# jiahuei/COMIC-Compact-Image-Captioning-with-Attention

Hardware: AMD Instinct MI355X
Metric: images/sec (decoder-mode XE training, COMIC-256, InceptionV3 frozen) (higher is better)
Workload: dtype bf16

## Files before the change

### comic-compact-image-captioning-with-attention_amd/_lib.py

```python
import ctypes as C
import os

_HERE = os.path.dirname(os.path.abspath(__file__))
LIB_PATH = os.environ.get('COMIC_HIP_LIB') or os.path.join(_HERE, 'lib', 'libcomic_hip.so')

c_void_p, c_int, c_int32, c_int64, c_float, c_double, c_char_p, c_uint64 = (
    C.c_void_p, C.c_int, C.c_int32, C.c_int64, C.c_float, C.c_double, C.c_char_p, C.c_uint64)


class CnnOp(C.Structure):
    _fields_ = [(n, c_int32) for n in (
        'kind', 'src', 'dst', 'src_coff', 'dst_coff', 'H', 'W', 'Cin', 'Cout', 'KH', 'KW', 'SH', 'SW',
        'PT', 'PL', 'Ho', 'Wo', 'weight', 'relu', 'out_f32', 'src_f32', 'lane', 'tile', 'group', 'flags', 'min_lds')]


class ImageDesc(C.Structure):
    _fields_ = [('offset', C.c_int64), ('in_h', c_int32), ('in_w', c_int32), ('flip', c_int32), ('oy', c_int32),
                ('ox', c_int32), ('sy', C.c_float), ('sx', C.c_float)]


class ConvWeight(C.Structure):
    _fields_ = [('w', c_void_p), ('scale', c_void_p), ('shift', c_void_p), ('w_frag', c_void_p)]


# ... 7 lines not shown
        'init_method', 'start_id', 'end_id')] + [(n, c_float) for n in (
            'keep_in', 'keep_out', 'keep_alpha', 'map_loss_scale')] + [('flags', C.c_uint32),
                                                                       ('length_penalty_weight', c_float),
                                                                       ('cell', c_int32)]


CELLS = {'LSTM': 0, 'LN_LSTM': 1, 'GRU': 2}


(DEC_NO_PERSIST, DEC_NO_PERSIST_BWD, DEC_NO_FUSED_STEP, DEC_NO_SPLIT_ATTN_BWD, DEC_ONE_LANE, DEC_EXACT_GEMM, DEC_STAMPS,
 DEC_NO_BEAM_LOGITS, DEC_NO_LSTM_STREAM) = (1, 2, 4, 8, 16, 32, 64, 128, 256)
DEC_PHASE_FWD, DEC_PHASE_BWD = 512, 1024
DEC_NO_GROUP_GEMM = 2048
DEC_BWD_OWN_ROWS = 4096
DEC_INJECT_TIMEOUT = 8192
CNN_BWD_NO_ACT_FUSION = 2
_DEC_ENV = (('COMIC_PERSIST', '0', DEC_NO_PERSIST), ('COMIC_PERSIST_BWD', '0', DEC_NO_PERSIST_BWD),
            ('COMIC_FUSED_STEP', '0', DEC_NO_FUSED_STEP), ('COMIC_SPLIT_ATTN_BWD', '0', DEC_NO_SPLIT_ATTN_BWD),
            ('COMIC_GRAD_LANES', '0', DEC_ONE_LANE), ('COMIC_SPLIT3', '0', DEC_EXACT_GEMM),
            ('COMIC_PERSIST_STAMPS', '1', DEC_STAMPS), ('COMIC_BEAM_LOGITS', '0', DEC_NO_BEAM_LOGITS),
            ('COMIC_LSTM_STREAM', '0', DEC_NO_LSTM_STREAM), ('COMIC_GROUP_GEMM', '0', DEC_NO_GROUP_GEMM),
            ('COMIC_BWD_OWN_ROWS', '1', DEC_BWD_OWN_ROWS))


def decoder_flags_from_env():
    f = 0
    for name, val, bit in _DEC_ENV:
        if os.environ.get(name, '')[:1] == val:
            f |= bit
    return f
# ... 77 lines not shown
    'comic_xent_fwd_bwd': (c_int, [P, P, P, P, P, P, P, P, c_int, c_int, c_int, P]),
    'comic_argmax_rows': (c_int, [P, P, c_int, c_int, P]),
    'comic_beam_step': (c_int, [P, P, P, P, P, P, P, c_int, c_int, c_int, c_int, P]),
    'comic_gather_rows': (c_int, [P, P, P, c_int, c_int, c_int, P]),
    'comic_gather_tree': (c_int, [P, P, P, P, c_int, c_int, c_int, c_int, P]),
    'comic_adam_tf': (c_int, [P, P, P, P, c_int64, c_float, c_float, c_float, c_float, c_float, c_float, P]),
    'comic_adam_tf_gated': (c_int, [P, P, P, P, c_int64, c_float, c_float, c_float, c_float, c_float, c_float, P, P]),
    'comic_momentum_tf_gated': (c_int, [P, P, P, c_int64, c_float, c_float, c_float, c_float, P, P]),
    'comic_debug_occupy_cus': (c_int, [c_int, c_int, P]),
    'comic_colsum': (c_int, [P, P, c_int, c_int, c_float, P]),
    'comic_ln_tanh_fwd': (c_int, [P, P, P, P, P, c_int, c_int, c_float, P]),
    'comic_ln_tanh_bwd_rows': (c_int, [P, P, P, P, P, c_int, c_int, P]),
    'comic_momentum_tf': (c_int, [P, P, P, c_int64, c_float, c_float, c_float, c_float, P]),
    'comic_axpy': (c_int, [P, P, c_float, c_int64, P]),
    'comic_decoder_train_workspace': (c_int64, [P, c_int, c_int]),
    'comic_decoder_train_path': (c_int, []),
    'comic_decoder_greedy_path': (c_int, []),
    'comic_decoder_beam_path': (c_int, []),
    'comic_beam_step_dense_workspace': (c_int64, [c_int, c_int, c_int, c_int]),
    'comic_beam_step_dense': (c_int, [c_void_p] * 9 + [c_int] * 5 + [c_void_p, c_int64, c_void_p]),
    'comic_gemm_f32_stream_workspace': (c_int64, [c_int, c_int, c_int]),
    'comic_gemm_f32_stream': (c_int, [c_void_p, c_void_p, c_void_p, c_void_p, c_int, c_int, c_int, c_void_p, c_int64, c_void_p]),
    'comic_decoder_infer_workspace': (c_int64, [P, c_int, c_int]),
    'comic_decoder_train_step': (c_int, [P, P, P, P, P, P, P, P, P, P, c_int, c_int, c_int, P, P, P, P, P, P, P,
                                         P, P, P, P, P, c_int64, P]),
    'comic_decoder_greedy': (c_int, [P, P, P, P, c_int, c_int, P, P, P, P, P, c_int64, P]),
    'comic_decoder_sample': (c_int, [P, P, P, P, c_int, c_int, P, P, P, P, P, P, c_int64, P]),
    'comic_decoder_beam': (c_int, [P, P, P, P, c_int, c_int, c_int, P, P, P, P, P, P, P, P, c_int64, P]),
    'comic_scorer_create': (c_void_p, [c_char_p, P, c_int64, c_double]),
    'comic_scorer_destroy': (None, [c_void_p]),
# ... 106 lines not shown
```

### comic-compact-image-captioning-with-attention_amd/csrc/decoder_exec.hip

```cpp
#include <atomic>
#include <stdlib.h>

#include <algorithm>
#include <string.h>

#include "common.h"
#include "decoder_math.h"
#include "decoder_persist.h"
#include "gemm_group.h"
#include "lstm_prep.h"
#include "lstm_stream_dev.h"

int comic_gemm_f32_ws(const float* A, const float* B, float* C, const float* bias, int M, int N, int K, int lda,
                      int ldb, int ldc, int trans_a, int trans_b, float alpha, float beta, void* ws, int64_t ws_bytes,
                      hipStream_t st);
int comic_xent_ex(float* logits, const int32_t* targets_bt, const float* coef_bt, const float* wmask_bt,
                  const int32_t* lens, float* loss_rows, float* dlogits, int32_t* ids_tb, int t_rows, int t_stride,
                  int B, int V, hipStream_t st);

int comic_attn_fwd_ex(const comic_attn_desc* d, const float* keys, const float* values, const float* q,
                      const float* ln_g, const float* ln_b, const float* v, const float* tau, const float* mask_alpha,
                      float keep_alpha, float* alpha, float* alpha_d, float* ctx, const int32_t* lens, int t,
                      const float* att_prev, float* att_next, float* xh_next, int xh_ld, const float* mask_next,
                      int mask_ld, float keep_in, int q_parts, float* q_out, float* scores_ws, hipStream_t st,
// ... 770 lines not shown
  w.take<unsigned>(kPersistSyncWords + kGroupTickets);
  w.take<float>(TB * 4 * D); w.take<float>((long)T * ((B + 15) / 16) * 16 * 4 * D);
  w.take<float>((long)T * ((B + 15) / 16) * 16 * D);
  w.take<float>(TB * 2 * D);
  w.take<float>(4 * B * (3 * D + 1));
  w.take<float>(TB * 64);
  if (comic_persist_fwd_bigm((int)M, d->fm_projection == 2)) w.take<float>(TB * 8 * M);
  if (d->cell == COMIC_CELL_LN_LSTM) {
    w.take<float>((TB + B) * 5 * D); w.take<float>((TB + B) * 8); w.take<float>((TB + B) * 10 * D); w.take<float>(10 * D);
  } else if (d->cell == COMIC_CELL_GRU) {
    w.take<float>(TB * Wd); w.take<float>(2 * B * Wd); w.take<float>(4 * D);
  }
  return (int64_t)w.off;
}

extern "C" int comic_decoder_train_step(const comic_decoder_desc* d, const comic_decoder_params* p,
                                        const comic_decoder_params* gr, const float* fm, const float* im_embed,
                                        const int32_t* inputs_bt, const int32_t* targets_bt, const float* wmask_bt,
                                        const float* coef_bt, const int32_t* lens, int B, int T, int Tp,
                                        const float* mask_init_in, const float* mask_in, const float* mask_out,
                                        const float* mask_alpha, float* logits_tb, int32_t* ids_tb, float* attn_hist,
                                        float* loss_rows, float* map_loss, float* dfm, float* dim_embed,
                                        void* workspace, int64_t workspace_bytes, void* stream) {
  RC(check_desc(d));
  FlagScope flag_scope__(d);
  COMIC_REQUIRE(p && gr && fm && im_embed && inputs_bt && targets_bt && wmask_bt && coef_bt && lens,
                "train_step: null input");
  COMIC_REQUIRE(logits_tb && ids_tb && attn_hist && loss_rows && map_loss && workspace, "train_step: null output");
  COMIC_REQUIRE(B > 0 && T > 0 && Tp > 0 && Tp <= T, "train_step: bad B/T/Tp (%d %d %d)", B, T, Tp);
  COMIC_REQUIRE(workspace_bytes >= comic_decoder_train_workspace(d, B, T), "train_step: workspace too small");
  COMIC_REQUIRE(d->keep_in >= 1.f || (mask_in && (d->init_method == 1 || mask_init_in)),
                "train_step: input dropout enabled but no mask given");
  COMIC_REQUIRE(d->keep_out >= 1.f || mask_out, "train_step: output dropout enabled but no mask given");
  COMIC_REQUIRE(d->keep_alpha >= 1.f || mask_alpha, "train_step: attention dropout enabled but no mask given");
  hipStream_t st = (hipStream_t)stream;
  const int D = d->D, E = d->E, A = d->A, V = d->V, M = d->M, H = d->H, Cv = d->Cv, EA = E + A, Wd = E + A + D;
  const long TB = (long)T * B;
  const bool drop_in = d->keep_in < 1.f, drop_out = d->keep_out < 1.f, drop_al = d->keep_alpha < 1.f;
  Bump w(workspace, (size_t)workspace_bytes);
  float* keys = w.take<float>((long)B * M * D);
  float* values_buf = w.take<float>((long)B * M * D);
  InitBufs ib;
  ib.x = w.take<float>((long)B * EA); ib.xh = w.take<float>((long)B * EA);
  ib.g = w.take<float>((long)B * 4 * D); ib.gates = w.take<float>((long)B * 4 * D); ib.c_new = w.take<float>((long)B * D);
  float* emb_all = w.take<float>(TB * E);
// ... 82 lines not shown
    if (persist_b) {
      pr.p[3] = dq_part; pr.n[3] = (long)Tp * B * 4 * D;
      pr.p[4] = dg_blk; pr.n[4] = 4 * n16;
      pr.p[5] = dstate; pr.n[5] = (long)Tp * B * 2 * D;
      pr.p[6] = dq_sum; pr.n[6] = n16;
      pr.p[7] = dotp; pr.n[7] = (long)Tp * B * 64;
    }
    ComicPrologueExtra px{};
    prologue_rides = group_gemm_enabled() && cell == COMIC_CELL_LSTM && fused;
    if (prologue_rides) {
      px.K = p->K; px.panel = kpanel_f; px.D = D; px.Wd = Wd; px.n_pack = comic_lstm_panel_floats(D, Wd, 0);
      if (Vp != V) { px.W_o = p->W_o; px.wo_pad = wo_pad; px.V = V; px.Vp = Vp; px.n_pad = (long)D * Vp; }
    }
    RC(comic_persist_prepare(pr, persist_sync, kPersistSyncWords + kGroupTickets, st, prologue_rides ? &px : nullptr));
  }
  const bool grp = group_gemm_enabled() && cell == COMIC_CELL_LSTM && (long)Tp * B >= 64 && (long)B * M >= 64 && B >= 16;
  const int ldl = grp ? Vp : V;
  const float* wo_g = (grp && Vp != V) ? wo_pad : p->W_o;
  float* xh_init = xh_all + (size_t)Tp * B * Wd;
  float* dg_init = dg_all + (size_t)Tp * B * 4 * D;
  void* const gg_slab = g_splitk_ws;
  const int64_t gg_slab_cap = 2 * kSplitKBytes;
  SideLane* L = grp ? nullptr : side_lane();
  if (do_fwd) {
  if (grp) {
    if (!persist) COMIC_REQUIRE(hipMemsetAsync(gg_tickets, 0, sizeof(unsigned) * kGroupTickets, st) == hipSuccess, "train_step: memset");
    if (fused && !(prologue_rides && persist_b)) RC(comic_pack_lstm_panels(p->K, prologue_rides ? nullptr : kpanel_f, persist_b ? nullptr : kpanel_b, D, Wd, st));
    if (fused_q && !persist_b) RC(comic_pack_wq_panel(p->W_q, wq_panel, D, st));
    if (Vp != V && !prologue_rides) {
      const long n = (long)D * Vp;
      hipLaunchKernelGGL(pad_rows_kernel, dim3((unsigned)cdiv64(n, 256)), dim3(256), 0, st, p->W_o, wo_pad, V, Vp, n);
      COMIC_LAUNCH_CHECK("pad W_o");
    }
    GemmGroupRun g1;
    g1.add(COMIC_GG_NN, fm, p->W_m, keys, B * M, D, d->C, d->C, D, D);
    if (d->fm_projection == 1) g1.add(COMIC_GG_NN, fm, p->W_v, values_buf, B * M, D, d->C, d->C, D, D);
    if (d->init_method == 1) {
      g1.add(COMIC_GG_NN, im_embed, p->W_init, hs, B, D, d->Cg, d->Cg, D, D);
    } else {
      ComicGemmProb* q = g1.add(COMIC_GG_NN, im_embed, p->W_init, xh_init, B, EA, d->Cg, d->Cg, EA, Wd);
      if (drop_in) { q->mask = mask_init_in; q->ld_mask = EA; q->keep = d->keep_in; }
    }
    RC(g1.run(gg_slab, gg_slab_cap, gg_tickets, st));
    if (d->init_method == 1) {
      RC(fill(cs, 0.f, (long)B * D, st));
    } else {
      GemmGroupRun g2;
      g2.add(COMIC_GG_NN, xh_init, p->K, ib.g, B, 4 * D, EA, Wd, 4 * D, 4 * D)->bias = p->b;
      RC(g2.run(gg_slab, gg_slab_cap, gg_tickets, st));
    }
  } else {
    LaneScope lane(L, st, splitk_ws_b);
    RC(lane.rc);
    hipStream_t sl = lane.lane();
    if (fused) RC(comic_pack_lstm_panels(p->K, kpanel_f, persist_b ? nullptr : kpanel_b, D, Wd, sl));
// ... 239 lines not shown
      hipLaunchKernelGGL(input_bwd_kernel, dim3(cdiv(B * Wd, 256)), dim3(256), 0, st, part,
                         drop_in ? mask_in + (size_t)t * B * EA : nullptr, d->keep_in, demb + (size_t)t * B * E,
                         datt, dh, lens, t, carry, B, E, A, D, S4);
      COMIC_LAUNCH_CHECK("input_bwd");
    }
  }
  float* dx_im = nullptr;
  int n_init = 0;
  if (grp) {
    const bool init_step = d->init_method != 1;
    const int rows_k = (Tp + (init_step ? 1 : 0)) * B;
    if (init_step)
      RC(comic_lstm_gates_bwd(ib.gates, nullptr, ib.c_new, nullptr, nullptr, 1.f, nullptr, 0, dc, dh, dg_init, B, D, (void*)st));
    GemmGroupRun g1, g2;
    g1.add(COMIC_GG_TN, xh_all, dg_all, gr->K, Wd, 4 * D, rows_k, Wd, 4 * D, 4 * D);
    g1.add(COMIC_GG_TN, fm, dkeys, gr->W_m, d->C, D, B * M, d->C, D, D);
    if (d->fm_projection == 1) g1.add(COMIC_GG_TN, fm, dvalues_buf, gr->W_v, d->C, D, B * M, d->C, D, D);
    if (persist_b) {
      ComicGemmProb* q = g1.add(COMIC_GG_NT, dg_all, p->K, demb, Tp * B, E, 4 * D, 4 * D, 4 * D, E);
      if (drop_in) { q->mask = mask_in; q->ld_mask = EA; q->keep = d->keep_in; }
    }
    g1.add(COMIC_GG_TN, y_all, dq_all, gr->W_q, D, D, Tp * B, D, D, D);
    g1.add(COMIC_GG_TN, y_all, dlogits, gr->W_o, D, V, Tp * B, D, ldl, V);
    if (dfm) g1.add(COMIC_GG_NT, dkeys, p->W_m, dfm, B * M, d->C, D, D, D, d->C);
    g1.add_colsum(dg_all, gr->b, 4 * D, rows_k, 4 * D);
    g1.add_colsum(dlogits, gr->b_o, V, Tp * B, ldl);
    if (d->method == 0) {
      const float* pg = persist_b ? pgrad4 : pgrad;
      const int pr = persist_b ? 4 * B : Tp * B, ldp = 3 * D + 1;
      g1.add_colsum(pg, gr->v, D, pr, ldp);
      g1.add_colsum(pg + D, gr->ln_g, D, pr, ldp);
      g1.add_colsum(pg + 2 * D, gr->ln_b, D, pr, ldp);
      g1.add_colsum(pg + 3 * D, gr->tau, 1, pr, ldp);
    }
    if (init_step) {
      ComicGemmProb* q = g1.add(COMIC_GG_NT, dg_init, p->K, dx_init, B, EA, 4 * D, 4 * D, 4 * D, EA);
      if (drop_in) { q->mask = mask_init_in; q->ld_mask = EA; q->keep = d->keep_in; }
      dx_im = dx_init;
      n_init = EA;
      g2.add(COMIC_GG_TN, im_embed, dx_im, gr->W_init, d->Cg, n_init, B, d->Cg, n_init, n_init);
      if (dim_embed) g2.add(COMIC_GG_NT, dx_im, p->W_init, dim_embed, B, d->Cg, n_init, n_init, n_init, d->Cg);
    } else {
      dx_im = dh;
      n_init = D;
      g1.add(COMIC_GG_TN, im_embed, dx_im, gr->W_init, d->Cg, n_init, B, d->Cg, n_init, n_init);
      if (dim_embed) g1.add(COMIC_GG_NT, dx_im, p->W_init, dim_embed, B, d->Cg, n_init, n_init, n_init, d->Cg);
    }
    if (d->fm_projection == 1 && dfm) {
      ComicGemmProb* q = g2.add(COMIC_GG_NT, dvalues_buf, p->W_v, dfm, B * M, d->C, D, D, D, d->C);
      q->beta = 1.f;
    }
    RC(g1.run(gg_slab, gg_slab_cap, gg_tickets, st));
    RC(comic_embed_bwd_set(in_tb, demb, gr->emb, Tp * B, E, V, st));
    RC(g2.run(gg_slab, gg_slab_cap, gg_tickets, st));
    if (d->fm_projection == 0 && dfm) RC(comic_axpy(dfm, dvalues_buf, 1.f, (int64_t)B * M * Cv, (void*)st));
  } else {
  LaneScope glane(L, st, splitk_ws_b);
  RC(glane.rc);
  hipStream_t sb = glane.lane();
  RC(gemm_big(y_all, dlogits, gr->W_o, nullptr, D, V, Tp * B, D, V, V, 1, 0, 0.f, sb));
// ... 531 lines not shown
```

### comic-compact-image-captioning-with-attention_amd/csrc/gemm_group.h

```cpp
#pragma once
#include "common.h"

constexpr int kGemmGroupMax = 20;
enum { COMIC_GG_TN = 0, COMIC_GG_NN = 1, COMIC_GG_NT = 2 };

struct ComicGemmProb {
  const float* A;
  const float* B;
  float* C;
  const float* bias;
  const float* mask;
  int M, N, K, lda, ldb, ldc, ld_mask;
  float alpha, beta;
  float keep;
  int type;
  int ones_a;
  int tiles_m, tiles_n, S, k_per_slice, wg_begin;
  int slab_tile0;
  int ticket0;
};

struct ComicGemmGroup {
  ComicGemmProb p[kGemmGroupMax];
  int n;
  float* slab;
  unsigned* tickets;
  int xcd_chunk;
};

int comic_gemm_group_plan(ComicGemmGroup& g, int target_items, int64_t* slab_bytes, int* n_tickets);
constexpr int kGemmGroupTargetItems = 640;
// ... 2 lines not shown
```

### comic-compact-image-captioning-with-attention_amd/csrc/gemm_group.hip

```cpp
#include <algorithm>

#include "gemm_group.h"
#include "gemm_x3_dev.h"

namespace {

constexpr int GB = 128;
constexpr int kGemmGroupSlots = 512;
constexpr int kItemOverhead = 6;
constexpr int kSc1 = 16;
typedef __attribute__((ext_vector_type(4))) unsigned gg_u32x4_t;

__device__ __forceinline__ __amdgpu_buffer_rsrc_t gg_rsrc(const void* p, long bytes) {
  return __builtin_amdgcn_make_buffer_rsrc((void*)p, 0, (int)bytes, 0x00020000);
}
__device__ __forceinline__ float4 gg_load16_sc1(__amdgpu_buffer_rsrc_t r, unsigned off) {
  const gg_u32x4_t v = __builtin_amdgcn_raw_buffer_load_b128(r, (int)off, 0, kSc1);
  return make_float4(__uint_as_float(v.x), __uint_as_float(v.y), __uint_as_float(v.z), __uint_as_float(v.w));
}
__device__ __forceinline__ void gg_store16_sc1(__amdgpu_buffer_rsrc_t r, unsigned off, float4 v) {
  const gg_u32x4_t u = {__float_as_uint(v.x), __float_as_uint(v.y), __float_as_uint(v.z), __float_as_uint(v.w)};
  __builtin_amdgcn_raw_buffer_store_b128(u, r, (int)off, 0, kSc1);
}

// ... 67 lines not shown
    red[kg * 32 + cg] = sm;
    __syncthreads();
    if (tid < 32) {
      float4 tot = red[cg];
#pragma unroll
      for (int k = 1; k < KG; ++k) {
        const float4 v = red[k * 32 + cg];
        tot.x += v.x; tot.y += v.y; tot.z += v.z; tot.w += v.w;
      }
      if (S == 1) gg_emit(p, 0, n, tot);
      else gg_store16_sc1(sr, sbase + (unsigned)cg * 16u, tot);
    }
    if (S == 1) return;
  } else {
    f32x4_t acc[4][4];
    if constexpr (PC) {
      if (p.type == COMIC_GG_TN) x3_mainloop_pc<false, false>(p.A, p.B, p.M, p.N, p.lda, p.ldb, m0, n0, kbeg, kend, smem, acc);
      else if (p.type == COMIC_GG_NN) x3_mainloop_pc<true, false>(p.A, p.B, p.M, p.N, p.lda, p.ldb, m0, n0, kbeg, kend, smem, acc);
      else x3_mainloop_pc<true, true>(p.A, p.B, p.M, p.N, p.lda, p.ldb, m0, n0, kbeg, kend, smem, acc);
    } else {
      if (p.type == COMIC_GG_TN)
        x3_mainloop<GB, false, false, GB>(p.A, p.B, p.M, p.N, p.lda, p.ldb, m0, n0, kbeg, kend, smem, acc);
      else if (p.type == COMIC_GG_NN)
        x3_mainloop<GB, true, false, GB>(p.A, p.B, p.M, p.N, p.lda, p.ldb, m0, n0, kbeg, kend, smem, acc);
      else
        x3_mainloop<GB, true, true, GB>(p.A, p.B, p.M, p.N, p.lda, p.ldb, m0, n0, kbeg, kend, smem, acc);
    }
    const bool owner = wave < 4;
    if (S == 1) {
      if (owner)
#pragma unroll
      for (int i = 0; i < 4; ++i)
#pragma unroll
        for (int j = 0; j < 4; ++j)
          gg_emit(p, m0 + wm * 64 + j * 16 + (lane & 15), n0 + wn * 64 + i * 16 + (lane >> 4) * 4,
                  make_float4(acc[i][j][0], acc[i][j][1], acc[i][j][2], acc[i][j][3]));
      return;
    }
    if (owner)
#pragma unroll
    for (int i = 0; i < 4; ++i)
// ... 35 lines not shown
    }
  }
}


}

int comic_gemm_group_plan(ComicGemmGroup& g, int target_items, int64_t* slab_bytes, int* n_tickets) {
  COMIC_REQUIRE(g.n > 0 && g.n <= kGemmGroupMax, "gemm_group: %d problems", g.n);
  long cost = 0;
  for (int i = 0; i < g.n; ++i) {
    ComicGemmProb& p = g.p[i];
    COMIC_REQUIRE(p.M > 0 && p.N > 0 && p.K > 0 && p.B && p.C && (p.A || p.ones_a), "gemm_group: bad problem %d", i);
    COMIC_REQUIRE(p.type >= COMIC_GG_TN && p.type <= COMIC_GG_NT, "gemm_group: bad type of problem %d", i);
    COMIC_REQUIRE(!p.ones_a || (p.type == COMIC_GG_TN && p.M == 1), "gemm_group: ones_a needs type TN and M = 1 (problem %d)", i);
    COMIC_REQUIRE(p.ldc >= p.N && (!p.mask || p.ld_mask >= p.N), "gemm_group: leading dimension of problem %d", i);
    if (!p.ones_a) COMIC_REQUIRE(p.lda >= (p.type == COMIC_GG_TN ? p.M : p.K), "gemm_group: lda of problem %d", i);
    COMIC_REQUIRE(p.ldb >= (p.type == COMIC_GG_NT ? p.K : p.N), "gemm_group: ldb of problem %d", i);
    p.tiles_m = cdiv(p.M, GB);
    p.tiles_n = cdiv(p.N, GB);
    cost += (long)cdiv(p.M, GB) * p.tiles_n * cdiv(p.K, 32);
  }
  auto split_of = [](int kt, long klen) { return (int)std::min<long>(16, std::max<long>(1, (kt + klen / 2) / klen)); };
  long klen = std::max<long>(8, cost / std::max(1, target_items));
  {
    long best = -1, best_klen = klen, kt_max = 8;
    for (int i = 0; i < g.n; ++i) kt_max = std::max<long>(kt_max, cdiv(g.p[i].K, 32));
    for (long kl = klen; kl <= kt_max; ++kl) {
      long items = 0, longest = 0;
      for (int i = 0; i < g.n; ++i) {
// ... 29 lines not shown
  }
  if (slab_bytes) *slab_bytes = (int64_t)slab_tiles * GB * GB * 4;
  if (n_tickets) *n_tickets = tickets;
  return wg;
}

int comic_gemm_group_launch(const ComicGemmGroup& g_in, int n_wg, hipStream_t st) {
  ComicGemmGroup g = g_in;
  g.xcd_chunk = n_wg / 8;
  COMIC_REQUIRE(n_wg > 0, "gemm_group: empty launch");
  bool pc = n_wg <= 256;
  for (int i = 0; i < g.n && pc; ++i) {
    const ComicGemmProb& p = g.p[i];
    if (p.ones_a) continue;
    const bool a_kc = p.type != COMIC_GG_TN, b_kc = p.type == COMIC_GG_NT;
    pc = p.lda % 4 == 0 && p.ldb % 4 == 0 && ((uintptr_t)p.A & 15) == 0 && ((uintptr_t)p.B & 15) == 0 &&
         (!(a_kc || b_kc) || p.K % 4 == 0);
  }
  static PerDeviceOnce once, once_pc;
  bool& done = pc ? once_pc.slot() : once.slot();
  const int lds = pc ? kGroupLdsPc : kGroupLds;
  if (!done) {
    const void* fn = pc ? (const void*)gemm_group_x3_kernel<true> : (const void*)gemm_group_x3_kernel<false>;
    COMIC_REQUIRE(hipFuncSetAttribute(fn, hipFuncAttributeMaxDynamicSharedMemorySize, lds) == hipSuccess,
                  "gemm_group: cannot reserve %d bytes of LDS", lds);
    done = true;
  }
  if (pc) hipLaunchKernelGGL(gemm_group_x3_kernel<true>, dim3((unsigned)n_wg), dim3(512), lds, st, g);
  else hipLaunchKernelGGL(gemm_group_x3_kernel<false>, dim3((unsigned)n_wg), dim3(256), lds, st, g);
  COMIC_LAUNCH_CHECK("gemm_group");
  return 0;
// ... 43 lines not shown
```

### comic-compact-image-captioning-with-attention_amd/decoder.py

```python
from __future__ import annotations

import ctypes as C
import math
from dataclasses import dataclass

import numpy as np

from . import _lib as L
from .ops import number_to_base

STEP_SCOPE = 'decoder/multi_head_attention_wrapper_v3/'
TF_NAMES = {
    'W_init': {'first_input': 'rnn_init_input/projection/weight', 'project_hidden': 'rnn_initial_state/weight'},
    'K': 'basic_lstm_cell/kernel', 'b': 'basic_lstm_cell/bias',
    'W_m': 'memory_layer/kernel', 'W_v': 'value_layer/kernel',
    'W_q': 'multi_add_attention/query_layer/kernel', 'v': 'multi_add_attention/attention_v',
    'ln_g': 'multi_add_attention/LN_tanh/gamma', 'ln_b': 'multi_add_attention/LN_tanh/beta',
    'tau': 'softmax_temperature', 'W_a': 'a_layer/kernel',
    'W_o': 'output_projection/kernel', 'b_o': 'output_projection/bias', 'emb': 'embedding_map',
    'K_c': 'gru_cell/candidate/kernel', 'b_c': 'gru_cell/candidate/bias',
}
STEP_VARS = ('W_q', 'v', 'ln_g', 'ln_b', 'tau', 'W_a')
CELL_SCOPES = {'LSTM': ('basic_lstm_cell', 'kernel', 'bias'), 'LN_LSTM': ('layer_norm_basic_lstm_cell', 'kernel', None),
               'GRU': ('gru_cell', 'gates/kernel', 'gates/bias')}
# ... 194 lines not shown
def process_inputs(captions, token_type):
    sent = np.asarray(captions, np.int64)
    masks = np.sign((sent[:, 1:] + 1).astype(np.float32))
    lens = masks.sum(axis=1).astype(np.int32)
    if token_type == 'word':
        sent = np.maximum(sent, 0)
        inputs = sent[:, :-1]
    else:
        inputs = sent[:, :-1]
        sent = np.maximum(sent, 0)
    targets = sent[:, 1:]
    return (np.ascontiguousarray(inputs, np.int32), np.ascontiguousarray(targets, np.int32),
            np.ascontiguousarray(masks, np.float32), lens)


class Decoder:

    def __init__(self, spec: DecoderSpec, params: dict | None = None, device='cuda:0', seed=0):
        import torch
        self.torch = torch
        self.lib = L.load()
        self.spec, self.device = spec, device
        self.params = FlatParams(spec.param_shapes(), device, status_tail=True)
        self.params.load(params if params is not None else init_params(spec, seed))
        self.grads = self.params.like()
        self._ws = None
        self._ws_bytes = 0
        self._dropout_calls = 0
        self.set_dropout_stream(seed, 0)
        self._ctx = {}
# ... 23 lines not shown
                    'dropout_mask')
            off += t.numel()
            out[name] = t
        return out

    def _train_ctx(self, B, T, Tp, training, gen_masks, want_input_grads):
        key = (B, T, Tp, bool(training), bool(gen_masks), bool(want_input_grads))
        ctx = self._ctx.get(key)
        if ctx is not None:
            return ctx
        torch, s, dev = self.torch, self.spec, self.device
        from types import SimpleNamespace
        ctx = SimpleNamespace(key=key, calls=0, graph=None)
        f32 = dict(dtype=torch.float32, device=dev)
        n_i32, n_f32 = 2 * B * T + B, 3 * B * T
        o_i32, o_f32 = 8, 8 + 4 * ((n_i32 + 1) // 2 * 2)
        nbytes = o_f32 + 4 * n_f32

        def views(buf):
            return (buf[:8].view(torch.int64), buf[o_i32:o_i32 + 4 * n_i32].view(torch.int32),
                    buf[o_f32:o_f32 + 4 * n_f32].view(torch.float32))
        ctx.stage_dev = torch.zeros(nbytes, dtype=torch.uint8, device=dev)
        ctx.seed, ctx.i32, ctx.f32 = views(ctx.stage_dev)
        ctx.stage = []
        for _ in range(2):
            buf = torch.zeros(nbytes, dtype=torch.uint8).pin_memory()
            sd, i32, f32v = views(buf)
            ctx.stage.append(SimpleNamespace(buf=buf, seed=sd, i32=i32, f32=f32v, copied=None))
        ctx.fm = torch.empty((B, s.M, s.C), **f32)
        ctx.im = torch.empty((B, s.Cg), **f32)
        EA = s.E + s.A
        ctx.masks = None
        if training:
            shapes = dict(init_in=(B, EA), inp=(Tp, B, EA), out=(Tp, B, s.D), alpha=(Tp, B, s.H, s.M))
            sizes = [int(np.prod(v)) for v in shapes.values()]
            ctx.mask_buf = torch.empty(sum(sizes), **f32)
            ctx.masks, off = {}, 0
            for (k, shp), n in zip(shapes.items(), sizes):
                ctx.masks[k] = ctx.mask_buf[off:off + n].view(shp)
                off += n
            ctx.mask_n4 = (C.c_int64 * 4)(*sizes)
            ctx.mask_keep4 = (C.c_float * 4)(1 - s.dropout_rnn_in, 1 - s.dropout_rnn_in, 1 - s.dropout_rnn_out,
                                             s.attn_keep_prob)
# ... 25 lines not shown
        st = L.stream_ptr()
        m = ctx.masks or {}
        if training and gen_masks and phase != 'bwd':
            L.check(self.lib.comic_dropout_masks4_dev(ctx.mask_buf.data_ptr(), ctx.mask_n4, ctx.mask_keep4,
                                                      ctx.seed.data_ptr(), st), 'dropout_masks4')
            if s.recurrent_dropout:
                row_in = m['inp'][0, 0].clone()
                row_out = m['out'][0, 0].clone()
                m['inp'].copy_(row_in.expand_as(m['inp']))
                m['init_in'].copy_(row_in.expand_as(m['init_in']))
                m['out'].copy_(row_out.expand_as(m['out']))
        BT = B * T
        i32, f32 = ctx.i32, ctx.f32
        ptab, gtab = self.params.table(), self.grads.table()
        ctx.desc.flags = (L.decoder_flags_from_env() | {None: 0, 'fwd': L.DEC_PHASE_FWD, 'bwd': L.DEC_PHASE_BWD}[phase]
                          | (L.DEC_INJECT_TIMEOUT if ctx.__dict__.pop('inject_timeout', False) else 0))
        L.check(self.lib.comic_decoder_train_step(
            C.byref(ctx.desc), C.byref(ptab), C.byref(gtab), ctx.fm_in.data_ptr(), ctx.im_in.data_ptr(),
            i32.data_ptr(), i32.data_ptr() + 4 * BT, f32.data_ptr(), f32.data_ptr() + 4 * BT,
            i32.data_ptr() + 8 * BT, B, T, Tp,
            L.ptr(m.get('init_in')), L.ptr(m.get('inp')), L.ptr(m.get('out')), L.ptr(m.get('alpha')),
            ctx.logits.data_ptr(), ctx.ids.data_ptr(), ctx.hist.data_ptr(), ctx.loss_rows.data_ptr(),
            ctx.map_loss.data_ptr(), L.ptr(ctx.dfm), L.ptr(ctx.dim), ctx.ws.data_ptr(), ctx.nbytes, st),
            'decoder_train_step')
        if phase == 'fwd':
            return
        L.check(self.lib.comic_weighted_sum_tb(ctx.loss_rows.data_ptr(), f32.data_ptr() + 4 * 2 * BT, T, B,
                                               ctx.loss.data_ptr(), st), 'weighted_sum_tb')

    def train_step(self, fm, im_embed, captions, masks=None, rewards=None, training=True, seed=None,
                   want_input_grads=False, xe_denom=None, use_graph=False, on_inputs_consumed=None, dp=None,
                   copy_inputs=True, phase=None, inject_timeout=False):
        torch, s = self.torch, self.spec
# ... 19 lines not shown
            slot = ctx.stage[(ctx.calls - 1) % 2]
            slot.copied.synchronize()
            fh = slot.f32.numpy()
            fh[BT:2 * BT] = coef.reshape(-1); fh[2 * BT:] = rs.reshape(-1)
            ctx.stage_dev.copy_(slot.buf, non_blocking=True)
            slot.copied.record(torch.cuda.current_stream())
            self._run_train_phase(ctx, 'bwd', use_graph)
            return dict(loss=ctx.loss[0], map_loss=ctx.map_loss[0], logits=ctx.logits.permute(1, 0, 2), ids=ctx.ids.t(),
                        attn_maps=ctx.hist.permute(1, 2, 0, 3), dfm=ctx.dfm, dim_embed=ctx.dim, Tp=Tp)
        slot = ctx.stage[ctx.calls % 2]
        if slot.copied is not None:
            slot.copied.synchronize()
        ih, fh = slot.i32.numpy(), slot.f32.numpy()
        ih[:BT] = inputs.reshape(-1); ih[BT:2 * BT] = targets.reshape(-1); ih[2 * BT:] = lens
        fh[:BT] = wmask.reshape(-1); fh[BT:2 * BT] = coef.reshape(-1); fh[2 * BT:] = rs.reshape(-1)
        if gen_masks:
            if seed is None:
                self._dropout_calls += 1
                seed = (self._dropout_base + self._dropout_calls) & 0x7FFFFFFFFFFFFFFF
            slot.seed[0] = int(seed)
        ctx.stage_dev.copy_(slot.buf, non_blocking=True)
        if masks is not None:
            for k, v in masks.items():
                ctx.masks[k].copy_(v if torch.is_tensor(v) else torch.from_numpy(np.ascontiguousarray(v, np.float32)))
        if dp is not None and dp.world > 1 and rewards is None:
            f = ctx.f32
            inv = 1.0 / dp.global_xe_denominator(f[:BT])
            torch.mul(f[:BT], inv, out=f[BT:2 * BT])
            f[2 * BT:3 * BT] = inv
        if slot.copied is None:
            slot.copied = torch.cuda.Event()
        slot.copied.record(torch.cuda.current_stream())
        assert fm.shape == (B, s.M, s.C) and im_embed.shape == (B, s.Cg), (fm.shape, im_embed.shape)
        assert fm.dtype == torch.float32 and im_embed.dtype == torch.float32
        direct = (not copy_inputs and not use_graph and fm.is_contiguous() and im_embed.is_contiguous())
        if direct:
            ctx.fm_in, ctx.im_in = fm, im_embed
        else:
            ctx.fm.copy_(fm)
            ctx.im.copy_(im_embed)
            ctx.fm_in, ctx.im_in = ctx.fm, ctx.im
            if on_inputs_consumed is not None:
                on_inputs_consumed()
        if phase == 'fwd':
            ctx.split_open = True
            self._run_train_phase(ctx, 'fwd', use_graph)
            if direct and on_inputs_consumed is not None:
                on_inputs_consumed()
            ctx.calls += 1
            return None
        if inject_timeout:
            assert not use_graph and phase is None
            ctx.inject_timeout = True
        if use_graph and ctx.graph is None and ctx.calls >= 1:
            g = torch.cuda.CUDAGraph()
            with torch.cuda.graph(g, capture_error_mode='thread_local'):
                self._train_device(ctx)
            ctx.graph = g
        if use_graph and ctx.graph is not None:
            ctx.graph.replay()
        else:
            self._train_device(ctx)
        if direct and on_inputs_consumed is not None:
            on_inputs_consumed()
        ctx.calls += 1
        return dict(loss=ctx.loss[0], map_loss=ctx.map_loss[0], logits=ctx.logits.permute(1, 0, 2), ids=ctx.ids.t(),
                    attn_maps=ctx.hist.permute(1, 2, 0, 3), dfm=ctx.dfm, dim_embed=ctx.dim, Tp=Tp)

    def _run_train_phase(self, ctx, phase, use_graph):
        torch = self.torch
        graphs = ctx.__dict__.setdefault('phase_graphs', {})
        used = ctx.__dict__.setdefault('phase_calls', {})
        used[phase] = used.get(phase, 0) + 1
# ... 221 lines not shown
```

### include/comic_hip.h

```cpp
#ifndef COMIC_HIP_H_
#define COMIC_HIP_H_

#include <stddef.h>
#include <stdint.h>

#ifdef __cplusplus
extern "C" {
#endif

#define COMIC_F32 0
#define COMIC_BF16 1
#define COMIC_F16 2
#define COMIC_ABI_VERSION 1
#define COMIC_CONV_TILES 61
#define COMIC_WS_TILE 54
#define COMIC_IMG_TILE 55
#define COMIC_CHAIN_TILE 62

const char* comic_last_error(void);
int comic_abi_version(void);
int comic_device_count(void);


int comic_pack_conv_weights(const float* w_hwio, void* w_packed, int kh, int kw, int cin, int cout,
// ... 220 lines not shown
} comic_decoder_desc;
#define COMIC_CELL_LSTM 0
#define COMIC_CELL_LN_LSTM 1
#define COMIC_CELL_GRU 2
#define COMIC_DEC_NO_PERSIST 1u
#define COMIC_DEC_NO_PERSIST_BWD 2u
#define COMIC_DEC_NO_FUSED_STEP 4u
#define COMIC_DEC_NO_SPLIT_ATTN_BWD 8u
#define COMIC_DEC_ONE_LANE 16u
#define COMIC_DEC_EXACT_GEMM 32u
#define COMIC_DEC_STAMPS 64u
#define COMIC_DEC_PHASE_FWD 512u
#define COMIC_DEC_PHASE_BWD 1024u
#define COMIC_DEC_NO_GROUP_GEMM 2048u
#define COMIC_DEC_INJECT_TIMEOUT 8192u
#define COMIC_DEC_BWD_OWN_ROWS 4096u
#define COMIC_DEC_NO_LSTM_STREAM 256u
#define COMIC_DEC_NO_BEAM_LOGITS 128u

typedef struct comic_decoder_params {
  float *W_init, *K, *b, *W_m, *W_v, *W_q, *v, *ln_g, *ln_b, *tau, *W_a, *W_o, *b_o, *emb;
  float* cell_ln;
  float *K_c, *b_c;
  float* status;
} comic_decoder_params;

int64_t comic_decoder_train_workspace(const comic_decoder_desc* d, int B, int T);
int64_t comic_decoder_infer_workspace(const comic_decoder_desc* d, int rows, int max_steps);

int comic_decoder_train_step(const comic_decoder_desc* d, const comic_decoder_params* p,
                             const comic_decoder_params* grads, const float* fm,
                             const float* im_embed, const int32_t* inputs_bt,
                             const int32_t* targets_bt, const float* wmask_bt, const float* coef_bt,
                             const int32_t* lens, int B, int T, int Tp, const float* mask_init_in,
                             const float* mask_in, const float* mask_out, const float* mask_alpha,
                             float* logits_tb, int32_t* ids_tb, float* attn_hist, float* loss_rows,
                             float* map_loss, float* dfm, float* dim_embed, void* workspace,
                             int64_t workspace_bytes, void* stream);

int comic_decoder_train_path(void);
int comic_decoder_greedy_path(void);
int comic_decoder_beam_path(void);

int comic_decoder_greedy(const comic_decoder_desc* d, const comic_decoder_params* p, const float* fm,
                         const float* im_embed, int B, int max_steps, int32_t* ids_tb,
                         float* logits_tb, float* attn_hist, int32_t* first_eos, void* workspace,
                         int64_t workspace_bytes, void* stream);

int comic_decoder_sample(const comic_decoder_desc* d, const comic_decoder_params* p, const float* fm,
                         const float* im_embed, int B, int max_steps, const float* gumbel_tb, int32_t* ids_tb,
                         float* logits_tb, float* attn_hist, int32_t* first_eos, void* workspace,
                         int64_t workspace_bytes, void* stream);

int comic_decoder_beam(const comic_decoder_desc* d, const comic_decoder_params* p, const float* fm,
// ... 20 lines not shown
```

Before: 39070.

## Read decoder fm/im_embed inputs through device address words under graph replay

When the training step is replayed as a captured graph, the grouped GEMMs now read the feature map and image embedding through a pointer stored in a small device staging word. The pointers are refreshed each call by the existing staged host-to-device copy. This lets graph replay consume caller tensors in place instead of first copying fm and im_embed into fixed graph buffers. The cost is an extra dependent pointer load per GEMM tile, alignment requirements, and relaxed alignment assumptions on the packed-copy path.

```diff
diff --git a/comic-compact-image-captioning-with-attention_amd/_lib.py b/comic-compact-image-captioning-with-attention_amd/_lib.py
--- a/comic-compact-image-captioning-with-attention_amd/_lib.py
+++ b/comic-compact-image-captioning-with-attention_amd/_lib.py
@@ -45,6 +45,7 @@
 DEC_NO_GROUP_GEMM = 2048
 DEC_BWD_OWN_ROWS = 4096
 DEC_INJECT_TIMEOUT = 8192
+DEC_INPUTS_INDIRECT = 16384
 CNN_BWD_NO_ACT_FUSION = 2
 _DEC_ENV = (('COMIC_PERSIST', '0', DEC_NO_PERSIST), ('COMIC_PERSIST_BWD', '0', DEC_NO_PERSIST_BWD),
             ('COMIC_FUSED_STEP', '0', DEC_NO_FUSED_STEP), ('COMIC_SPLIT_ATTN_BWD', '0', DEC_NO_SPLIT_ATTN_BWD),
@@ -152,6 +153,7 @@
     'comic_momentum_tf': (c_int, [P, P, P, c_int64, c_float, c_float, c_float, c_float, P]),
     'comic_axpy': (c_int, [P, P, c_float, c_int64, P]),
     'comic_decoder_train_workspace': (c_int64, [P, c_int, c_int]),
+    'comic_decoder_train_inputs_indirect': (c_int, [P, c_int, c_int]),
     'comic_decoder_train_path': (c_int, []),
     'comic_decoder_greedy_path': (c_int, []),
     'comic_decoder_beam_path': (c_int, []),
diff --git a/comic-compact-image-captioning-with-attention_amd/csrc/decoder_exec.hip b/comic-compact-image-captioning-with-attention_amd/csrc/decoder_exec.hip
--- a/comic-compact-image-captioning-with-attention_amd/csrc/decoder_exec.hip
+++ b/comic-compact-image-captioning-with-attention_amd/csrc/decoder_exec.hip
@@ -808,6 +808,15 @@
   return (int64_t)w.off;
 }
 
+static bool train_grouped(const comic_decoder_desc* d, uint32_t flags, int B, int Tp) {
+  return !(flags & (COMIC_DEC_NO_GROUP_GEMM | COMIC_DEC_EXACT_GEMM)) && d->cell == COMIC_CELL_LSTM && (long)Tp * B >= 64 &&
+         (long)B * d->M >= 64 && B >= 16;
+}
+
+extern "C" int comic_decoder_train_inputs_indirect(const comic_decoder_desc* d, int B, int Tp) {
+  return d && B > 0 && Tp > 0 && d->fm_projection != 0 && train_grouped(d, d->flags, B, Tp) ? 1 : 0;
+}
+
 extern "C" int comic_decoder_train_step(const comic_decoder_desc* d, const comic_decoder_params* p,
                                         const comic_decoder_params* gr, const float* fm, const float* im_embed,
                                         const int32_t* inputs_bt, const int32_t* targets_bt, const float* wmask_bt,
@@ -823,6 +832,10 @@
   COMIC_REQUIRE(logits_tb && ids_tb && attn_hist && loss_rows && map_loss && workspace, "train_step: null output");
   COMIC_REQUIRE(B > 0 && T > 0 && Tp > 0 && Tp <= T, "train_step: bad B/T/Tp (%d %d %d)", B, T, Tp);
   COMIC_REQUIRE(workspace_bytes >= comic_decoder_train_workspace(d, B, T), "train_step: workspace too small");
+  const int ind = (d->flags & COMIC_DEC_INPUTS_INDIRECT) ? 1 : 0;
+  COMIC_REQUIRE(!ind || comic_decoder_train_inputs_indirect(d, B, Tp),
+                "train_step: COMIC_DEC_INPUTS_INDIRECT needs the grouped products and a projected memory");
+  COMIC_REQUIRE(!ind || (((uintptr_t)fm | (uintptr_t)im_embed) & 7) == 0, "train_step: misaligned address word");
   COMIC_REQUIRE(d->keep_in >= 1.f || (mask_in && (d->init_method == 1 || mask_init_in)),
                 "train_step: input dropout enabled but no mask given");
   COMIC_REQUIRE(d->keep_out >= 1.f || mask_out, "train_step: output dropout enabled but no mask given");
@@ -935,7 +948,7 @@
     }
     RC(comic_persist_prepare(pr, persist_sync, kPersistSyncWords + kGroupTickets, st, prologue_rides ? &px : nullptr));
   }
-  const bool grp = group_gemm_enabled() && cell == COMIC_CELL_LSTM && (long)Tp * B >= 64 && (long)B * M >= 64 && B >= 16;
+  const bool grp = train_grouped(d, g_dec_flags, B, Tp);
   const int ldl = grp ? Vp : V;
   const float* wo_g = (grp && Vp != V) ? wo_pad : p->W_o;
   float* xh_init = xh_all + (size_t)Tp * B * Wd;
@@ -954,12 +967,13 @@
       COMIC_LAUNCH_CHECK("pad W_o");
     }
     GemmGroupRun g1;
-    g1.add(COMIC_GG_NN, fm, p->W_m, keys, B * M, D, d->C, d->C, D, D);
-    if (d->fm_projection == 1) g1.add(COMIC_GG_NN, fm, p->W_v, values_buf, B * M, D, d->C, d->C, D, D);
+    g1.add(COMIC_GG_NN, fm, p->W_m, keys, B * M, D, d->C, d->C, D, D)->a_indirect = ind;
+    if (d->fm_projection == 1) g1.add(COMIC_GG_NN, fm, p->W_v, values_buf, B * M, D, d->C, d->C, D, D)->a_indirect = ind;
     if (d->init_method == 1) {
-      g1.add(COMIC_GG_NN, im_embed, p->W_init, hs, B, D, d->Cg, d->Cg, D, D);
+      g1.add(COMIC_GG_NN, im_embed, p->W_init, hs, B, D, d->Cg, d->Cg, D, D)->a_indirect = ind;
     } else {
       ComicGemmProb* q = g1.add(COMIC_GG_NN, im_embed, p->W_init, xh_init, B, EA, d->Cg, d->Cg, EA, Wd);
+      q->a_indirect = ind;
       if (drop_in) { q->mask = mask_init_in; q->ld_mask = EA; q->keep = d->keep_in; }
     }
     RC(g1.run(gg_slab, gg_slab_cap, gg_tickets, st));
@@ -1229,8 +1243,8 @@
       RC(comic_lstm_gates_bwd(ib.gates, nullptr, ib.c_new, nullptr, nullptr, 1.f, nullptr, 0, dc, dh, dg_init, B, D, (void*)st));
     GemmGroupRun g1, g2;
     g1.add(COMIC_GG_TN, xh_all, dg_all, gr->K, Wd, 4 * D, rows_k, Wd, 4 * D, 4 * D);
-    g1.add(COMIC_GG_TN, fm, dkeys, gr->W_m, d->C, D, B * M, d->C, D, D);
-    if (d->fm_projection == 1) g1.add(COMIC_GG_TN, fm, dvalues_buf, gr->W_v, d->C, D, B * M, d->C, D, D);
+    g1.add(COMIC_GG_TN, fm, dkeys, gr->W_m, d->C, D, B * M, d->C, D, D)->a_indirect = ind;
+    if (d->fm_projection == 1) g1.add(COMIC_GG_TN, fm, dvalues_buf, gr->W_v, d->C, D, B * M, d->C, D, D)->a_indirect = ind;
     if (persist_b) {
       ComicGemmProb* q = g1.add(COMIC_GG_NT, dg_all, p->K, demb, Tp * B, E, 4 * D, 4 * D, 4 * D, E);
       if (drop_in) { q->mask = mask_in; q->ld_mask = EA; q->keep = d->keep_in; }
@@ -1253,12 +1267,12 @@
       if (drop_in) { q->mask = mask_init_in; q->ld_mask = EA; q->keep = d->keep_in; }
       dx_im = dx_init;
       n_init = EA;
-      g2.add(COMIC_GG_TN, im_embed, dx_im, gr->W_init, d->Cg, n_init, B, d->Cg, n_init, n_init);
+      g2.add(COMIC_GG_TN, im_embed, dx_im, gr->W_init, d->Cg, n_init, B, d->Cg, n_init, n_init)->a_indirect = ind;
       if (dim_embed) g2.add(COMIC_GG_NT, dx_im, p->W_init, dim_embed, B, d->Cg, n_init, n_init, n_init, d->Cg);
     } else {
       dx_im = dh;
       n_init = D;
-      g1.add(COMIC_GG_TN, im_embed, dx_im, gr->W_init, d->Cg, n_init, B, d->Cg, n_init, n_init);
+      g1.add(COMIC_GG_TN, im_embed, dx_im, gr->W_init, d->Cg, n_init, B, d->Cg, n_init, n_init)->a_indirect = ind;
       if (dim_embed) g1.add(COMIC_GG_NT, dx_im, p->W_init, dim_embed, B, d->Cg, n_init, n_init, n_init, d->Cg);
     }
     if (d->fm_projection == 1 && dfm) {
diff --git a/comic-compact-image-captioning-with-attention_amd/csrc/gemm_group.h b/comic-compact-image-captioning-with-attention_amd/csrc/gemm_group.h
--- a/comic-compact-image-captioning-with-attention_amd/csrc/gemm_group.h
+++ b/comic-compact-image-captioning-with-attention_amd/csrc/gemm_group.h
@@ -15,6 +15,7 @@
   float keep;
   int type;
   int ones_a;
+  int a_indirect;
   int tiles_m, tiles_n, S, k_per_slice, wg_begin;
   int slab_tile0;
   int ticket0;
diff --git a/comic-compact-image-captioning-with-attention_amd/csrc/gemm_group.hip b/comic-compact-image-captioning-with-attention_amd/csrc/gemm_group.hip
--- a/comic-compact-image-captioning-with-attention_amd/csrc/gemm_group.hip
+++ b/comic-compact-image-captioning-with-attention_amd/csrc/gemm_group.hip
@@ -105,17 +105,18 @@
     if (S == 1) return;
   } else {
     f32x4_t acc[4][4];
+    const float* const pA = p.a_indirect ? *(const float* const*)p.A : p.A;
     if constexpr (PC) {
-      if (p.type == COMIC_GG_TN) x3_mainloop_pc<false, false>(p.A, p.B, p.M, p.N, p.lda, p.ldb, m0, n0, kbeg, kend, smem, acc);
-      else if (p.type == COMIC_GG_NN) x3_mainloop_pc<true, false>(p.A, p.B, p.M, p.N, p.lda, p.ldb, m0, n0, kbeg, kend, smem, acc);
-      else x3_mainloop_pc<true, true>(p.A, p.B, p.M, p.N, p.lda, p.ldb, m0, n0, kbeg, kend, smem, acc);
+      if (p.type == COMIC_GG_TN) x3_mainloop_pc<false, false>(pA, p.B, p.M, p.N, p.lda, p.ldb, m0, n0, kbeg, kend, smem, acc);
+      else if (p.type == COMIC_GG_NN) x3_mainloop_pc<true, false>(pA, p.B, p.M, p.N, p.lda, p.ldb, m0, n0, kbeg, kend, smem, acc);
+      else x3_mainloop_pc<true, true>(pA, p.B, p.M, p.N, p.lda, p.ldb, m0, n0, kbeg, kend, smem, acc);
     } else {
       if (p.type == COMIC_GG_TN)
-        x3_mainloop<GB, false, false, GB>(p.A, p.B, p.M, p.N, p.lda, p.ldb, m0, n0, kbeg, kend, smem, acc);
+        x3_mainloop<GB, false, false, GB>(pA, p.B, p.M, p.N, p.lda, p.ldb, m0, n0, kbeg, kend, smem, acc);
       else if (p.type == COMIC_GG_NN)
-        x3_mainloop<GB, true, false, GB>(p.A, p.B, p.M, p.N, p.lda, p.ldb, m0, n0, kbeg, kend, smem, acc);
+        x3_mainloop<GB, true, false, GB>(pA, p.B, p.M, p.N, p.lda, p.ldb, m0, n0, kbeg, kend, smem, acc);
       else
-        x3_mainloop<GB, true, true, GB>(p.A, p.B, p.M, p.N, p.lda, p.ldb, m0, n0, kbeg, kend, smem, acc);
+        x3_mainloop<GB, true, true, GB>(pA, p.B, p.M, p.N, p.lda, p.ldb, m0, n0, kbeg, kend, smem, acc);
     }
     const bool owner = wave < 4;
     if (S == 1) {
@@ -181,6 +182,7 @@
     COMIC_REQUIRE(p.M > 0 && p.N > 0 && p.K > 0 && p.B && p.C && (p.A || p.ones_a), "gemm_group: bad problem %d", i);
     COMIC_REQUIRE(p.type >= COMIC_GG_TN && p.type <= COMIC_GG_NT, "gemm_group: bad type of problem %d", i);
     COMIC_REQUIRE(!p.ones_a || (p.type == COMIC_GG_TN && p.M == 1), "gemm_group: ones_a needs type TN and M = 1 (problem %d)", i);
+    COMIC_REQUIRE(!p.a_indirect || (!p.ones_a && ((uintptr_t)p.A & 7) == 0), "gemm_group: bad address word of problem %d", i);
     COMIC_REQUIRE(p.ldc >= p.N && (!p.mask || p.ld_mask >= p.N), "gemm_group: leading dimension of problem %d", i);
     if (!p.ones_a) COMIC_REQUIRE(p.lda >= (p.type == COMIC_GG_TN ? p.M : p.K), "gemm_group: lda of problem %d", i);
     COMIC_REQUIRE(p.ldb >= (p.type == COMIC_GG_NT ? p.K : p.N), "gemm_group: ldb of problem %d", i);
@@ -240,7 +242,7 @@
     const ComicGemmProb& p = g.p[i];
     if (p.ones_a) continue;
     const bool a_kc = p.type != COMIC_GG_TN, b_kc = p.type == COMIC_GG_NT;
-    pc = p.lda % 4 == 0 && p.ldb % 4 == 0 && ((uintptr_t)p.A & 15) == 0 && ((uintptr_t)p.B & 15) == 0 &&
+    pc = p.lda % 4 == 0 && p.ldb % 4 == 0 && (p.a_indirect || ((uintptr_t)p.A & 15) == 0) && ((uintptr_t)p.B & 15) == 0 &&
          (!(a_kc || b_kc) || p.K % 4 == 0);
   }
   static PerDeviceOnce once, once_pc;
diff --git a/comic-compact-image-captioning-with-attention_amd/decoder.py b/comic-compact-image-captioning-with-attention_amd/decoder.py
--- a/comic-compact-image-captioning-with-attention_amd/decoder.py
+++ b/comic-compact-image-captioning-with-attention_amd/decoder.py
@@ -232,6 +232,14 @@
             np.ascontiguousarray(masks, np.float32), lens)
 
 
+def inputs_in_place(fm, im_embed, use_graph, indirect):
+    if not (fm.is_contiguous() and im_embed.is_contiguous()):
+        return False
+    if not use_graph:
+        return True
+    return bool(indirect) and fm.data_ptr() % 16 == 0 and im_embed.data_ptr() % 16 == 0
+
+
 class Decoder:
 
     def __init__(self, spec: DecoderSpec, params: dict | None = None, device='cuda:0', seed=0):
@@ -285,19 +293,21 @@
         ctx = SimpleNamespace(key=key, calls=0, graph=None)
         f32 = dict(dtype=torch.float32, device=dev)
         n_i32, n_f32 = 2 * B * T + B, 3 * B * T
-        o_i32, o_f32 = 8, 8 + 4 * ((n_i32 + 1) // 2 * 2)
+        o_i32 = 24
+        o_f32 = o_i32 + 4 * ((n_i32 + 1) // 2 * 2)
         nbytes = o_f32 + 4 * n_f32
 
         def views(buf):
             return (buf[:8].view(torch.int64), buf[o_i32:o_i32 + 4 * n_i32].view(torch.int32),
-                    buf[o_f32:o_f32 + 4 * n_f32].view(torch.float32))
+                    buf[o_f32:o_f32 + 4 * n_f32].view(torch.float32), buf[8:24].view(torch.int64))
         ctx.stage_dev = torch.zeros(nbytes, dtype=torch.uint8, device=dev)
-        ctx.seed, ctx.i32, ctx.f32 = views(ctx.stage_dev)
+        ctx.seed, ctx.i32, ctx.f32, ctx.addr = views(ctx.stage_dev)
+        ctx.indirect = False
         ctx.stage = []
         for _ in range(2):
             buf = torch.zeros(nbytes, dtype=torch.uint8).pin_memory()
-            sd, i32, f32v = views(buf)
-            ctx.stage.append(SimpleNamespace(buf=buf, seed=sd, i32=i32, f32=f32v, copied=None))
+            sd, i32, f32v, addr = views(buf)
+            ctx.stage.append(SimpleNamespace(buf=buf, seed=sd, i32=i32, f32=f32v, addr=addr, copied=None))
         ctx.fm = torch.empty((B, s.M, s.C), **f32)
         ctx.im = torch.empty((B, s.Cg), **f32)
         EA = s.E + s.A
@@ -353,9 +363,12 @@
         i32, f32 = ctx.i32, ctx.f32
         ptab, gtab = self.params.table(), self.grads.table()
         ctx.desc.flags = (L.decoder_flags_from_env() | {None: 0, 'fwd': L.DEC_PHASE_FWD, 'bwd': L.DEC_PHASE_BWD}[phase]
-                          | (L.DEC_INJECT_TIMEOUT if ctx.__dict__.pop('inject_timeout', False) else 0))
+                          | (L.DEC_INJECT_TIMEOUT if ctx.__dict__.pop('inject_timeout', False) else 0)
+                          | (L.DEC_INPUTS_INDIRECT if ctx.indirect else 0))
+        fm_arg, im_arg = ((ctx.addr.data_ptr(), ctx.addr.data_ptr() + 8) if ctx.indirect
+                          else (ctx.fm_in.data_ptr(), ctx.im_in.data_ptr()))
         L.check(self.lib.comic_decoder_train_step(
-            C.byref(ctx.desc), C.byref(ptab), C.byref(gtab), ctx.fm_in.data_ptr(), ctx.im_in.data_ptr(),
+            C.byref(ctx.desc), C.byref(ptab), C.byref(gtab), fm_arg, im_arg,
             i32.data_ptr(), i32.data_ptr() + 4 * BT, f32.data_ptr(), f32.data_ptr() + 4 * BT,
             i32.data_ptr() + 8 * BT, B, T, Tp,
             L.ptr(m.get('init_in')), L.ptr(m.get('inp')), L.ptr(m.get('out')), L.ptr(m.get('alpha')),
@@ -405,6 +418,18 @@
         ih, fh = slot.i32.numpy(), slot.f32.numpy()
         ih[:BT] = inputs.reshape(-1); ih[BT:2 * BT] = targets.reshape(-1); ih[2 * BT:] = lens
         fh[:BT] = wmask.reshape(-1); fh[BT:2 * BT] = coef.reshape(-1); fh[2 * BT:] = rs.reshape(-1)
+        assert fm.shape == (B, s.M, s.C) and im_embed.shape == (B, s.Cg), (fm.shape, im_embed.shape)
+        assert fm.dtype == torch.float32 and im_embed.dtype == torch.float32
+        if use_graph and phase is None and ctx.graph is not None:
+            ctx.indirect = ctx.graph_indirect
+        else:
+            ctx.desc.flags = L.decoder_flags_from_env()
+            ctx.indirect = bool(use_graph and phase is None and not inject_timeout and
+                                self.lib.comic_decoder_train_inputs_indirect(C.byref(ctx.desc), B, Tp))
+        direct = not copy_inputs and inputs_in_place(fm, im_embed, use_graph, ctx.indirect)
+        if ctx.indirect:
+            src = (fm, im_embed) if direct else (ctx.fm, ctx.im)
+            slot.addr[0], slot.addr[1] = src[0].data_ptr(), src[1].data_ptr()
         if gen_masks:
             if seed is None:
                 self._dropout_calls += 1
@@ -422,9 +447,6 @@
         if slot.copied is None:
             slot.copied = torch.cuda.Event()
         slot.copied.record(torch.cuda.current_stream())
-        assert fm.shape == (B, s.M, s.C) and im_embed.shape == (B, s.Cg), (fm.shape, im_embed.shape)
-        assert fm.dtype == torch.float32 and im_embed.dtype == torch.float32
-        direct = (not copy_inputs and not use_graph and fm.is_contiguous() and im_embed.is_contiguous())
         if direct:
             ctx.fm_in, ctx.im_in = fm, im_embed
         else:
@@ -447,7 +469,7 @@
             g = torch.cuda.CUDAGraph()
             with torch.cuda.graph(g, capture_error_mode='thread_local'):
                 self._train_device(ctx)
-            ctx.graph = g
+            ctx.graph, ctx.graph_indirect = g, ctx.indirect
         if use_graph and ctx.graph is not None:
             ctx.graph.replay()
         else:
diff --git a/include/comic_hip.h b/include/comic_hip.h
--- a/include/comic_hip.h
+++ b/include/comic_hip.h
@@ -258,6 +258,7 @@
 #define COMIC_DEC_PHASE_BWD 1024u
 #define COMIC_DEC_NO_GROUP_GEMM 2048u
 #define COMIC_DEC_INJECT_TIMEOUT 8192u
+#define COMIC_DEC_INPUTS_INDIRECT 16384u
 #define COMIC_DEC_BWD_OWN_ROWS 4096u
 #define COMIC_DEC_NO_LSTM_STREAM 256u
 #define COMIC_DEC_NO_BEAM_LOGITS 128u
@@ -282,6 +283,8 @@
                              float* map_loss, float* dfm, float* dim_embed, void* workspace,
                              int64_t workspace_bytes, void* stream);
 
+int comic_decoder_train_inputs_indirect(const comic_decoder_desc* d, int B, int Tp);
+
 int comic_decoder_train_path(void);
 int comic_decoder_greedy_path(void);
 int comic_decoder_beam_path(void);
```

Result: no change. 39340, median of 2 (+0.7%).
